# ax-le/nn-fac

Hardware: AMD Instinct MI355X
Metric: HALS NMF outer iterations/s (100000x2000 rank-50 row blocks per second) (higher is better)
Workload: dtype f32; 1 GPU; NMF hals beta=2, 100000x2000 rank 50 per GPU (configs[1] of BASELINE.json), deterministic (alpha=inf, delta=0.01, maxiter=100); rows_total=100000, cols=2000, rank=50, rows_per_rank=100000, parallelism=single GPU, cost_evaluation=streaming kernel (nnf_frob_resid_f32)

## Files before the change

include/nnfac_hip.h:

```cpp
#ifndef NNFAC_HIP_H
#define NNFAC_HIP_H

#include <stddef.h>
#include <stdint.h>

#ifdef __cplusplus
extern "C" {
#endif

#define NNF_OK 0
#define NNF_ERR_ARG (-1)
#define NNF_ERR_LAUNCH (-2)
#define NNF_ERR_UNSUPPORTED (-3)
#define NNF_ERR_WORKSPACE (-4)
#define NNF_ERR_DEVICE (-5)

#define NNF_MAX_RANK 128

#define NNF_HALS_SPARSITY 1u
#define NNF_HALS_NORMALIZE 2u
#define NNF_HALS_NONZERO 4u

typedef struct nnf_ctx nnf_ctx;

// ... 4 lines not shown
#define NNF_HALS_ST_WORDS 8

int nnf_version(void);
size_t nnf_build_flags(char* buf, size_t cap);
const char* nnf_status_string(int status);

int nnf_ctx_create(nnf_ctx** out_ctx, int device, size_t workspace_bytes);
int nnf_ctx_destroy(nnf_ctx* ctx);
size_t nnf_ctx_workspace_bytes(const nnf_ctx* ctx);
int nnf_ctx_set_scratch(nnf_ctx* ctx, void* device_buf, size_t bytes);

int nnf_ctx_set_probe(nnf_ctx* ctx, void* ev_begin, void* ev_end);
#define NNF_PROBE_XTY 0
#define NNF_PROBE_XHT 1
#define NNF_PROBE_COST 2
#define NNF_PROBE_HALS 3
#define NNF_PROBE_MU_LEFT 4
#define NNF_PROBE_MU_RIGHT 5
#define NNF_PROBE_MTTKRP 6
#define NNF_PROBE_COUNT 7
int nnf_ctx_set_probe_kernel(nnf_ctx* ctx, int kernel_id);
int nnf_ctx_set_probe_ring(nnf_ctx* ctx, void* const* events, int npairs);
int nnf_ctx_probe_ring_count(const nnf_ctx* ctx);

typedef struct nnf_comm nnf_comm;
int nnf_comm_unique_id(void* id_out_128_bytes);
int nnf_comm_create(nnf_comm** out_comm, nnf_ctx* ctx, int nranks, int rank, const void* id_128_bytes);
int nnf_comm_destroy(nnf_comm* comm);
int nnf_comm_size(const nnf_comm* comm);
int nnf_comm_rank(const nnf_comm* comm);
int nnf_allreduce_f32(nnf_comm* comm, float* buf, int64_t count, void* stream);
int nnf_allreduce_f64(nnf_comm* comm, double* buf, int64_t count, void* stream);

int nnf_gram_f32(nnf_ctx* ctx, const float* A, int r, int64_t K, int64_t lda, float* G, int64_t ldg, void* stream);
int nnf_gram_f64_f32(nnf_ctx* ctx, const float* A, int r, int64_t K, int64_t lda, float* G, int64_t ldg, double* G64, void* stream);

int nnf_xht_f32(nnf_ctx* ctx, const float* X, int64_t m, int64_t n, int64_t ldx, const float* V, int r, int64_t ldv,
                float* out, int64_t ldo, void* stream);

int nnf_xty_f32(nnf_ctx* ctx, const float* X, int64_t m, int64_t n, int64_t ldx, const float* Ut, int r, int64_t ldu,
                float* out, int64_t ldo, void* stream);

int nnf_frob_resid_f32(nnf_ctx* ctx, const float* X, int64_t m, int64_t n, int64_t ldx, const float* Ut, int64_t ldu,
                       const float* V, int64_t ldv, int r, double* out_f64, void* stream);

int nnf_nmf_gram_cost_f32(nnf_ctx* ctx, const float* V, int64_t ldv, const float* UtM, int64_t ldm, const float* UtU, const float* UtU_b,
                          int64_t ldg, int r, int64_t n, const double* normx2_f64, double* out_f64, void* stream);
int nnf_nmf_gram_cost_cal_f32(nnf_ctx* ctx, const float* V, int64_t ldv, const float* UtM, int64_t ldm, const float* UtU,
                              const float* UtU_b, int64_t ldg, int r, int64_t n, const double* normx2_f64, double sigma_a,
                              double bias_a, double* out_f64, void* stream);
int nnf_nmf_gram_cost_g64_f32(nnf_ctx* ctx, const float* V, int64_t ldv, const float* UtM, int64_t ldm, const float* UtU,
                              const double* UtU64, int64_t ldg, int r, int64_t n, const double* normx2_f64, double sigma_a,
                              double bias_a, double sigma_g, double* out_f64, void* stream);

int nnf_hals_solve_f32(nnf_ctx* ctx, const float* UtM, int64_t ldm, const float* UtU, int64_t ldg, float* V, int64_t ldv,
                       int r, int64_t ncols, int max_sweeps, double delta, float sparsity, unsigned flags,
                       double* status_f64, void* stream);

int nnf_hals_solve_cross_f32(nnf_ctx* ctx, const float* UtM, int64_t ldm, const float* UtU_a, const float* UtU_b, int64_t ldg,
                             const float* V_in, int64_t ldvi, float* V_out, int64_t ldvo, int r, int64_t ncols, int max_sweeps,
                             double delta, float sparsity, unsigned flags, double* status_f64, void* stream);

int nnf_hals_solve_continue_f32(nnf_ctx* ctx, const float* UtM, int64_t ldm, const float* UtU, int64_t ldg, float* V,
                                int64_t ldv, int r, int64_t ncols, int sweeps_done, int max_sweeps, double delta,
                                float sparsity, unsigned flags, double* status_f64, void* stream);

int nnf_hals_sweeps_f32(nnf_ctx* ctx, const float* UtM, int64_t ldm, const float* UtU, int64_t ldg, float* V, int64_t ldv,
                        int r, int64_t ncols, int nsweeps, float sparsity, unsigned flags, double* nodelta_f64,
                        float* snapshots, int64_t snap_stride, void* stream);

int nnf_hals_sweeps_ex_f32(nnf_ctx* ctx, const float* UtM, int64_t ldm, const float* UtU, int64_t ldg, float* V, int64_t ldv,
                           int r, int64_t ncols, int nsweeps, int sweeps_done, float sparsity, unsigned flags,
                           double* nodelta_f64, float* snapshots, int64_t snap_stride, int snap_first, const float* resid_in,
                           float* resid_out, void* stream);
int nnf_hals_resid_floats(nnf_ctx* ctx, int r, int64_t ncols, int64_t* floats_out);

int nnf_hals_row_update_f32(nnf_ctx* ctx, const float* UtM, int64_t ldm, const float* UtU, int64_t ldg, float* V, int64_t ldv, int r,
                            int64_t ncols, int k, float sparsity, unsigned flags, double* out2_f64, void* stream);
int nnf_hals_row_scale_f32(nnf_ctx* ctx, float* V, int64_t ldv, int64_t ncols, int k, const double* normsq_f64, int64_t ncols_total,
                           void* stream);

int nnf_hals_resident_columns(nnf_ctx* ctx, int r, int64_t* columns_out);

int nnf_hals_stop_restore_f32(nnf_ctx* ctx, const double* sums_f64, int nsweeps, int head, int budget, double delta, float* V,
                              int64_t ldv, int r, int64_t ncols, const float* snapshots, int64_t snap_stride,
                              double* status_f64, void* stream);

int nnf_mu_left_f32(nnf_ctx* ctx, const float* X, int64_t m, int64_t n, int64_t ldx, const float* Ut, int64_t ldu,
                    const float* V, int64_t ldv, int r, double beta, float* Ut_out, int64_t lduo, void* stream);

int nnf_mu_left_kl_cost_f32(nnf_ctx* ctx, const float* X, int64_t m, int64_t n, int64_t ldx, const float* Ut, int64_t ldu,
                            const float* V, int64_t ldv, int r, float* Ut_out, int64_t lduo, double* cost_f64, void* stream);

int nnf_mu_right_f32(nnf_ctx* ctx, const float* X, int64_t m, int64_t n, int64_t ldx, const float* Ut, int64_t ldu,
                     const float* V, int64_t ldv, int r, double beta, float* V_out, int64_t ldvo, void* stream);

int nnf_mu_right_accum_f32(nnf_ctx* ctx, const float* X, int64_t m, int64_t n, int64_t ldx, const float* Ut, int64_t ldu,
                           const float* V, int64_t ldv, int r, double beta, float* num, int64_t ldnum, float* den,
                           int64_t ldden, double* den_vec_f64, void* stream);
int nnf_mu_apply_f32(nnf_ctx* ctx, const float* F, int64_t ldf, int r, int64_t cols, const float* num, int64_t ldnum,
                     const float* den, int64_t ldden, const double* den_vec_f64, double beta, float* out, int64_t ldo,
                     void* stream);

int nnf_mu_ratio_f32(nnf_ctx* ctx, const float* X, int64_t m, int64_t n, int64_t ldx, const float* Ut, int64_t ldu,
                     const float* V, int64_t ldv, int r, double beta, float* R1, float* R2, int64_t ldr, void* stream);

// ... 42 lines not shown
```

nn_fac_amd/_lib.py:

```python
import ctypes as C
import os

from .utils.errors import EngineError

_HERE = os.path.dirname(os.path.abspath(__file__))
LIB_PATH = os.environ.get("NNF_LIBRARY") or os.path.join(_HERE, "libnnfac_hip.so")

_i64, _i32, _u32 = C.c_int64, C.c_int, C.c_uint
_p, _f32, _f64 = C.c_void_p, C.c_float, C.c_double

SIGNATURES = {
    "nnf_version": (_i32, []),
    "nnf_build_flags": (C.c_size_t, [C.c_char_p, C.c_size_t]),
    "nnf_status_string": (C.c_char_p, [_i32]),
    "nnf_ctx_create": (_i32, [C.POINTER(_p), _i32, C.c_size_t]),
    "nnf_ctx_destroy": (_i32, [_p]),
    "nnf_ctx_workspace_bytes": (C.c_size_t, [_p]),
    "nnf_comm_unique_id": (_i32, [_p]),
    "nnf_comm_create": (_i32, [C.POINTER(_p), _p, _i32, _i32, _p]),
    "nnf_comm_destroy": (_i32, [_p]),
    "nnf_comm_size": (_i32, [_p]),
    "nnf_comm_rank": (_i32, [_p]),
    "nnf_allreduce_f32": (_i32, [_p, _p, _i64, _p]),
    "nnf_allreduce_f64": (_i32, [_p, _p, _i64, _p]),
    "nnf_gram_f32": (_i32, [_p, _p, _i32, _i64, _i64, _p, _i64, _p]),
    "nnf_xht_f32": (_i32, [_p, _p, _i64, _i64, _i64, _p, _i32, _i64, _p, _i64, _p]),
    "nnf_xty_f32": (_i32, [_p, _p, _i64, _i64, _i64, _p, _i32, _i64, _p, _i64, _p]),
    "nnf_ctx_set_scratch": (_i32, [_p, _p, C.c_size_t]),
    "nnf_frob_resid_f32": (_i32, [_p, _p, _i64, _i64, _i64, _p, _i64, _p, _i64, _i32, _p, _p]),
    "nnf_nmf_gram_cost_f32": (_i32, [_p, _p, _i64, _p, _i64, _p, _p, _i64, _i32, _i64, _p, _p, _p]),
    "nnf_nmf_gram_cost_cal_f32": (_i32, [_p, _p, _i64, _p, _i64, _p, _p, _i64, _i32, _i64, _p, _f64, _f64, _p, _p]),
    "nnf_nmf_gram_cost_g64_f32": (_i32, [_p, _p, _i64, _p, _i64, _p, _p, _i64, _i32, _i64, _p, _f64, _f64, _f64, _p, _p]),
    "nnf_gram_f64_f32": (_i32, [_p, _p, _i32, _i64, _i64, _p, _i64, _p, _p]),
    "nnf_hals_solve_f32": (_i32, [_p, _p, _i64, _p, _i64, _p, _i64, _i32, _i64, _i32, _f64, _f32, _u32, _p, _p]),
    "nnf_hals_solve_cross_f32": (_i32, [_p, _p, _i64, _p, _p, _i64, _p, _i64, _p, _i64, _i32, _i64, _i32, _f64, _f32, _u32, _p,
                                        _p]),
    "nnf_hals_solve_continue_f32": (_i32, [_p, _p, _i64, _p, _i64, _p, _i64, _i32, _i64, _i32, _i32, _f64, _f32, _u32, _p,
                                           _p]),
    "nnf_hals_resident_columns": (_i32, [_p, _i32, C.POINTER(_i64)]),
    "nnf_hals_row_update_f32": (_i32, [_p, _p, _i64, _p, _i64, _p, _i64, _i32, _i64, _i32, _f32, _u32, _p, _p]),
    "nnf_hals_row_scale_f32": (_i32, [_p, _p, _i64, _i64, _i32, _p, _i64, _p]),
    "nnf_hals_stop_restore_f32": (_i32, [_p, _p, _i32, _i32, _i32, _f64, _p, _i64, _i32, _i64, _p, _i64, _p, _p]),
    "nnf_hals_sweeps_f32": (_i32, [_p, _p, _i64, _p, _i64, _p, _i64, _i32, _i64, _i32, _f32, _u32, _p, _p, _i64, _p]),
    "nnf_hals_sweeps_ex_f32": (_i32, [_p, _p, _i64, _p, _i64, _p, _i64, _i32, _i64, _i32, _i32, _f32, _u32, _p, _p, _i64, _i32,
                                      _p, _p, _p]),
    "nnf_hals_resid_floats": (_i32, [_p, _i32, _i64, C.POINTER(_i64)]),
    "nnf_ctx_set_probe": (_i32, [_p, _p, _p]),
    "nnf_ctx_set_probe_kernel": (_i32, [_p, _i32]),
    "nnf_ctx_set_probe_ring": (_i32, [_p, C.POINTER(_p), _i32]),
    "nnf_ctx_probe_ring_count": (_i32, [_p]),
    "nnf_mu_left_f32": (_i32, [_p, _p, _i64, _i64, _i64, _p, _i64, _p, _i64, _i32, _f64, _p, _i64, _p]),
    "nnf_mu_left_kl_cost_f32": (_i32, [_p, _p, _i64, _i64, _i64, _p, _i64, _p, _i64, _i32, _p, _i64, _p, _p]),
    "nnf_mu_right_f32": (_i32, [_p, _p, _i64, _i64, _i64, _p, _i64, _p, _i64, _i32, _f64, _p, _i64, _p]),
    "nnf_mu_right_accum_f32": (_i32, [_p, _p, _i64, _i64, _i64, _p, _i64, _p, _i64, _i32, _f64, _p, _i64, _p, _i64, _p, _p]),
    "nnf_ttm3_f32": (_i32, [_p, _p, _i64, _i64, _i64, _p, _i64, _i32, _i32, _p, _p]),
    "nnf_ntd_core_pg_f32": (_i32, [_p, _p, _p, _p, _p, _p, _i32, _i32, _i32, _f64, _f64, _i32, _f64, _p, _p]),
    "nnf_mu_ratio_f32": (_i32, [_p, _p, _i64, _i64, _i64, _p, _i64, _p, _i64, _i32, _f64, _p, _p, _i64, _p]),
    "nnf_mu_apply_f32": (_i32, [_p, _p, _i64, _i32, _i64, _p, _i64, _p, _i64, _p, _f64, _p, _i64, _p]),
    "nnf_mu_left_num_f32": (_i32, [_p, _p, _i64, _i64, _i64, _p, _i64, _p, _i64, _i32, _p, _i64, _p]),
    "nnf_small_gemm_f32": (_i32, [_p, _p, _i64, _i32, _i32, _p, _i64, _i64, _p, _i64, _p]),
    "nnf_deep_kl_apply_f32": (_i32, [_p, _p, _i64, _i32, _i64, _p, _i64, _p, _p, _i64, _f64, _p, _i64, _p]),
    "nnf_betadiv_f32": (_i32, [_p, _p, _i64, _i64, _i64, _p, _i64, _p, _i64, _i32, _f64, _p, _p]),
    "nnf_mttkrp3_f32": (_i32, [_p, _p, _i64, _i64, _i64, _p, _i64, _p, _i64, _p, _i64, _i32, _i32, _p, _i64, _p]),
    "nnf_mttkrp3_from_partial_f32": (_i32, [_p, _p, _i64, _i64, _p, _i64, _i32, _i32, _p, _i64, _p]),
    "nnf_cp3_partial_cost_f32": (_i32, [_p, _p, _i64, _i64, _i64, _p, _i64, _p, _i64, _p, _i64, _i32, _p, _p, _p]),
    "nnf_cp3_betadiv_f32": (_i32, [_p, _p, _i64, _i64, _i64, _p, _i64, _p, _i64, _p, _i64, _i32, _f64, _p, _p]),
    "nnf_dot_f32": (_i32, [_p, _p, _i64, _p, _i64, _i64, _i64, _p, _p]),
    "nnf_hadamard_f32": (_i32, [_p, _p, _p, _p, _i64, _p]),
}

_lib = None


def load():
    global _lib
    if _lib is not None:
        return _lib
    if not os.path.exists(LIB_PATH):
        raise EngineError(
            f"{LIB_PATH} not found: build it with `python -c 'import __graft_entry__ as g; g.build()'` "
            "or `make -C nn_fac_amd/csrc -j8` (there is no CPU fallback)")
    try:
        lib = C.CDLL(LIB_PATH)
    except OSError as e:
        raise EngineError(f"cannot load {LIB_PATH}: {e}") from e
# ... 12 lines not shown
```

nn_fac_amd/csrc/nnf_api.hip:

```cpp
#include "nnf_internal.h"
#include <new>

#include <map>
#include <string>
#include <string.h>

extern "C" int nnf_version(void) { return 101; }

static std::map<std::string, std::string>& build_flag_registry() {
    static std::map<std::string, std::string> r;
    return r;
}
void nnf_register_build_flags(const char* unit, const char* flags) { build_flag_registry()[unit] = flags; }

extern "C" size_t nnf_build_flags(char* buf, size_t cap) {
    std::string all;
    for (const auto& kv : build_flag_registry()) {
        if (!all.empty()) all += "; ";
        all += kv.first + ": " + kv.second;
    }
    if (buf && cap > 0) {
        const size_t n = all.size() < cap - 1 ? all.size() : cap - 1;
        memcpy(buf, all.data(), n);
        buf[n] = 0;
// ... 114 lines not shown
    for (int64_t e = (int64_t)blockIdx.x * 256 + threadIdx.x; e < total; e += (int64_t)gridDim.x * 256) {
        const int64_t i = e / cols, j = e - i * cols;
        s += (double)A[i * lda + j] * (double)B[i * ldb + j];
    }
    const double t = nnf_block_sum_f64(s, red);
    if (threadIdx.x == 0) partial[blockIdx.x] = t;
}
__global__ __launch_bounds__(256) void nnf_sum_f64_kernel(const double* __restrict__ partial, int64_t count,
                                                          double* __restrict__ out) {
    __shared__ double red[4];
    double s = 0.0;
    for (int64_t e = threadIdx.x; e < count; e += 8 * 256) {
        double v[8];
#pragma unroll
        for (int u = 0; u < 8; ++u) v[u] = partial[e + 256 * u < count ? e + 256 * u : count - 1];
#pragma unroll
        for (int u = 0; u < 8; ++u) s += (e + 256 * u < count) ? v[u] : 0.0;
    }
    const double t = nnf_block_sum_f64(s, red);
    if (threadIdx.x == 0) out[0] = t;
}

extern "C" int nnf_dot_f32(nnf_ctx* ctx, const float* A, int64_t lda, const float* B, int64_t ldb, int64_t rows,
                           int64_t cols, double* out_f64, void* stream) {
    if (!ctx || !A || !B || !out_f64 || rows < 1 || cols < 1 || lda < cols || ldb < cols) return NNF_ERR_ARG;
    hipStream_t st = (hipStream_t)stream;
    int64_t grid = nnf_cdiv(rows * cols, 256 * 8);
    if (grid > 1024) grid = 1024;
    if (grid < 1) grid = 1;
    nnf_ws_cursor cur(ctx);
    double* partial = (double*)cur.take((size_t)grid * 8);
    if (!partial) return NNF_ERR_WORKSPACE;
    hipLaunchKernelGGL(nnf_dot_kernel, dim3((int)grid), dim3(256), 0, st, A, lda, B, ldb, rows, cols, partial);
    NNF_CHECK_LAUNCH();
    hipLaunchKernelGGL(nnf_sum_f64_kernel, dim3(1), dim3(256), 0, st, partial, grid, out_f64);
    NNF_CHECK_LAUNCH();
    return NNF_OK;
}

__global__ void nnf_hadamard_kernel(const float* __restrict__ A, const float* __restrict__ B, float* __restrict__ C,
                                    int64_t count) {
    for (int64_t e = (int64_t)blockIdx.x * blockDim.x + threadIdx.x; e < count; e += (int64_t)gridDim.x * blockDim.x)
        C[e] = A[e] * B[e];
}
extern "C" int nnf_hadamard_f32(nnf_ctx* ctx, const float* A, const float* B, float* C, int64_t count, void* stream) {
    if (!ctx || !A || !B || !C || count < 1) return NNF_ERR_ARG;
    int64_t grid = nnf_cdiv(count, 256);
    if (grid > 1024) grid = 1024;
    hipLaunchKernelGGL(nnf_hadamard_kernel, dim3((int)grid), dim3(256), 0, (hipStream_t)stream, A, B, C, count);
    NNF_CHECK_LAUNCH();
    return NNF_OK;
}

template <typename GT>
__global__ __launch_bounds__(256) void nnf_gram_cost_kernel(const float* __restrict__ V, int64_t ldv, const float* __restrict__ UtM,
                                                            int64_t ldm, const float* __restrict__ G, const float* __restrict__ G2,
                                                            const double* __restrict__ G64, int64_t ldg, int r, int64_t n,
                                                            double* __restrict__ partial, unsigned* __restrict__ ticket,
                                                            const double* __restrict__ normx2, double* __restrict__ out,
                                                            double sigma_a, double bias_a, int g_global, double sigma_g) {
    extern __shared__ __attribute__((aligned(16))) float gc_sh[];
    GT* gsh = reinterpret_cast<GT*>(gc_sh);
    const GT* gsrc = reinterpret_cast<const GT*>(std::is_same<GT, double>::value ? (const void*)G64 : (const void*)G);
    const GT* g = g_global ? gsrc : gsh;
    const int64_t gs = g_global ? (std::is_same<GT, double>::value ? (int64_t)r : ldg) : r;
    float* vc = gc_sh + (g_global ? (size_t)0 : (size_t)r * r * (sizeof(GT) / 4));
    __shared__ double red[4];
    __shared__ unsigned last;
    if (!g_global)
        for (int e = threadIdx.x; e < r * r; e += 256) {
            const int64_t o = (int64_t)(e / r) * ldg + (e % r);
            if constexpr (std::is_same<GT, double>::value) gsh[e] = G64[e];
            else gsh[e] = G2 ? G[o] * G2[o] : G[o];
        }
    const int tc = threadIdx.x >> 4, t = threadIdx.x & 15;
    const int64_t j = (int64_t)blockIdx.x * 16 + tc;
    for (int a = t; a < r; a += 16) vc[tc * r + a] = (j < n) ? V[(int64_t)a * ldv + j] : 0.f;
    __syncthreads();
    double pA = 0.0, pA2 = 0.0, pB = 0.0, pV2 = 0.0;
    if (j < n) {
        const float* vj = vc + tc * r;
        for (int a = t; a < r; a += 16) {
            const GT* ga = g + (size_t)a * gs;
            double ta = 0.0;
            if (g_global && G2 != nullptr) {
                const float* gb = G2 + (size_t)a * ldg;
                for (int b = 0; b < r; ++b) ta = __builtin_fma((double)((float)ga[b] * gb[b]), (double)vj[b], ta);
            } else
            for (int b = 0; b < r; ++b) ta = __builtin_fma((double)ga[b], (double)vj[b], ta);
            const double va = (double)vj[a], p = va * (double)UtM[(int64_t)a * ldm + j];
            pA += p;
            pA2 = __builtin_fma(p, p, pA2);
            pB = __builtin_fma(va, ta, pB);
            pV2 = __builtin_fma(va, va, pV2);
        }
    }
    const double sA = nnf_block_sum_f64(pA, red), sA2 = nnf_block_sum_f64(pA2, red), sB = nnf_block_sum_f64(pB, red),
                 sV2 = nnf_block_sum_f64(pV2, red);
    if (threadIdx.x == 0) {
        unsigned long long* o = reinterpret_cast<unsigned long long*>(partial) + (size_t)blockIdx.x * 4;
        const double vals[4] = {sA, sA2, sB, sV2};
        for (int i = 0; i < 4; ++i)
            __hip_atomic_store(o + i, __builtin_bit_cast(unsigned long long, vals[i]), __ATOMIC_RELAXED, __HIP_MEMORY_SCOPE_AGENT);
        const unsigned tk = __hip_atomic_fetch_add(ticket, 1u, __ATOMIC_ACQ_REL, __HIP_MEMORY_SCOPE_AGENT);
        last = (tk == gridDim.x - 1u) ? 1u : 0u;
    }
    __syncthreads();
    if (last == 0u) return;
    const int nwg = (int)gridDim.x;
    double s[4] = {0.0, 0.0, 0.0, 0.0};
    const unsigned long long* pp = reinterpret_cast<const unsigned long long*>(partial);
    for (int e = threadIdx.x; e < nwg; e += 256)
#pragma unroll
        for (int i = 0; i < 4; ++i)
            s[i] += __builtin_bit_cast(double, __hip_atomic_load(pp + (size_t)e * 4 + i, __ATOMIC_RELAXED, __HIP_MEMORY_SCOPE_AGENT));
    double tot[4];
#pragma unroll
    for (int i = 0; i < 4; ++i) tot[i] = nnf_block_sum_f64(s[i], red);
    float gm = 0.f;
    for (int e = threadIdx.x; e < r * r; e += 256) {
        float ge = (float)g[(size_t)(e / r) * gs + (e % r)];
        if (g_global && G2 != nullptr) ge *= G2[(size_t)(e / r) * ldg + (e % r)];
        gm = fmaxf(gm, fabsf(ge));
    }
    gm = fmaxf(gm, __shfl_xor(gm, 1, 64));
    gm = fmaxf(gm, __shfl_xor(gm, 2, 64));
    gm = fmaxf(gm, __shfl_xor(gm, 4, 64));
    gm = fmaxf(gm, __shfl_xor(gm, 8, 64));
    gm = fmaxf(gm, __shfl_xor(gm, 16, 64));
    gm = fmaxf(gm, __shfl_xor(gm, 32, 64));
    __shared__ float gmax[4];
    if ((threadIdx.x & 63) == 0) gmax[threadIdx.x >> 6] = gm;
    __syncthreads();
    if (threadIdx.x == 0) {
        gm = fmaxf(fmaxf(gmax[0], gmax[1]), fmaxf(gmax[2], gmax[3]));
        const double cost = normx2[0] - 2.0 * tot[0] + tot[2];
        const double sa = 2.0 * sigma_a * sqrt(tot[1]), sb = sigma_g * (double)gm * tot[3];
        const double est = 4.0 * sqrt(sa * sa + sb * sb) + 2.0 * 2.0 * bias_a * fabs(tot[0]);
        out[0] = cost;
        out[1] = (est <= 5e-4 * cost) ? 0.0 : 1.0;
        out[2] = est;
        __hip_atomic_store(ticket, 0u, __ATOMIC_RELAXED, __HIP_MEMORY_SCOPE_AGENT);
    }
}
static int gram_cost_launch(nnf_ctx* ctx, const float* V, int64_t ldv, const float* UtM, int64_t ldm, const float* UtU,
                            const float* UtU_b, const double* UtU64, int64_t ldg, int r, int64_t n, const double* normx2_f64,
                            double sigma_a, double bias_a, double sigma_g, double* out_f64, void* stream) {
    if (!ctx || !V || !UtM || !UtU || !normx2_f64 || !out_f64 || r < 1 || n < 1 || ldv < n || ldm < n || ldg < r) return NNF_ERR_ARG;
    if (!(sigma_a >= 0.0) || !(bias_a >= 0.0) || !(sigma_g >= 0.0)) return NNF_ERR_ARG;
    if (UtU64 != nullptr && UtU_b != nullptr) return NNF_ERR_ARG;
    const int g_global = r > NNF_MAX_RANK ? 1 : 0;
    hipStream_t st = (hipStream_t)stream;
    const int64_t nwg = nnf_cdiv(n, 16);
    if (nwg > (int64_t)1 << 24) return NNF_ERR_UNSUPPORTED;
    nnf_ws_cursor cur(ctx);
    double* partial = (double*)cur.take((size_t)nwg * 4 * 8);
    if (!partial) return NNF_ERR_WORKSPACE;
    unsigned* ticket = ctx->gc_ticket;
    if (!ticket) return NNF_ERR_WORKSPACE;
    const size_t shm = ((g_global ? (size_t)0 : (size_t)r * r * (UtU64 ? 2 : 1)) + (size_t)16 * r) * 4;
    if (shm > 150 * 1024) return NNF_ERR_UNSUPPORTED;
    if (UtU64) {
        static bool attr = false;
        if (!attr) {
            (void)hipFuncSetAttribute(reinterpret_cast<const void*>(&nnf_gram_cost_kernel<double>), hipFuncAttributeMaxDynamicSharedMemorySize,
                                      150 * 1024);
            attr = true;
        }
        hipLaunchKernelGGL(nnf_gram_cost_kernel<double>, dim3((int)nwg), dim3(256), shm, st, V, ldv, UtM, ldm, UtU, UtU_b, UtU64, ldg, r, n,
                           partial, ticket, normx2_f64, out_f64, sigma_a, bias_a, g_global, sigma_g);
    } else {
        static bool attr = false;
        if (!attr) {
            (void)hipFuncSetAttribute(reinterpret_cast<const void*>(&nnf_gram_cost_kernel<float>), hipFuncAttributeMaxDynamicSharedMemorySize,
                                      96 * 1024);
            attr = true;
        }
        hipLaunchKernelGGL(nnf_gram_cost_kernel<float>, dim3((int)nwg), dim3(256), shm, st, V, ldv, UtM, ldm, UtU, UtU_b, UtU64, ldg, r, n,
                           partial, ticket, normx2_f64, out_f64, sigma_a, bias_a, g_global, sigma_g);
    }
    NNF_CHECK_LAUNCH();
    return NNF_OK;
}
extern "C" int nnf_nmf_gram_cost_f32(nnf_ctx* ctx, const float* V, int64_t ldv, const float* UtM, int64_t ldm, const float* UtU,
                                     const float* UtU_b, int64_t ldg, int r, int64_t n, const double* normx2_f64, double* out_f64,
                                     void* stream) {
    return gram_cost_launch(ctx, V, ldv, UtM, ldm, UtU, UtU_b, nullptr, ldg, r, n, normx2_f64, 6e-8, 0.0, 4e-8, out_f64, stream);
}
extern "C" int nnf_nmf_gram_cost_cal_f32(nnf_ctx* ctx, const float* V, int64_t ldv, const float* UtM, int64_t ldm, const float* UtU,
                                         const float* UtU_b, int64_t ldg, int r, int64_t n, const double* normx2_f64, double sigma_a,
                                         double bias_a, double* out_f64, void* stream) {
    return gram_cost_launch(ctx, V, ldv, UtM, ldm, UtU, UtU_b, nullptr, ldg, r, n, normx2_f64, sigma_a, bias_a, 4e-8, out_f64, stream);
}
extern "C" int nnf_nmf_gram_cost_g64_f32(nnf_ctx* ctx, const float* V, int64_t ldv, const float* UtM, int64_t ldm, const float* UtU,
                                         const double* UtU64, int64_t ldg, int r, int64_t n, const double* normx2_f64, double sigma_a,
                                         double bias_a, double sigma_g, double* out_f64, void* stream) {
    if (!UtU64) return NNF_ERR_ARG;
    return gram_cost_launch(ctx, V, ldv, UtM, ldm, UtU, nullptr, UtU64, ldg, r, n, normx2_f64, sigma_a, bias_a, sigma_g, out_f64, stream);
}
```

nn_fac_amd/engine.py:

```python
import ctypes as C
import os
import threading

import torch

from . import _lib
from .utils import errors as err
from .utils.errors import EngineError

HALS_SPARSITY, HALS_NORMALIZE, HALS_NONZERO = 1, 2, 4
ST_EPS, ST_CNT, ST_EPS0, ST_ERR, ST_WORDS = 0, 1, 2, 3, 8

_engines = {}
_lock = threading.Lock()

MAX_RANK = 128


def check_rank(r, where):
    r = int(r)
    if r > MAX_RANK:
        raise EngineError(f"{where}: rank {r} is above the {MAX_RANK} the Tucker kernels (core contractions, core update) of "
                          f"nn_fac_amd are built for; nmf, ntf, hals_nnls_acc and mu_betadivmin take any rank")

# ... 56 lines not shown
            if out64.dtype != torch.float64 or not out64.is_contiguous() or out64.numel() < r * r or out64.device != A.device:
                raise EngineError("gram: out64 must be a contiguous float64 device tensor of r*r elements")
            _lib.check(self.lib.nnf_gram_f64_f32(self.ctx, _ptr(A), r, K, _ld(A), _ptr(G), _ld(G), _ptr(out64), self._stream()),
                       "nnf_gram_f64_f32")
            return G
        _lib.check(self.lib.nnf_gram_f32(self.ctx, _ptr(A), r, K, _ld(A), _ptr(G), _ld(G), self._stream()),
                   "nnf_gram_f32")
        return G

    def xht(self, X, V, out=None):
        _chk2d(X, "xht X"), _chk2d(V, "xht V")
        m, n = X.shape
        r = V.shape[0]
        if V.shape[1] != n:
            raise EngineError("xht: shape mismatch")
        O = out if out is not None else torch.empty((r, m), dtype=torch.float32, device=X.device)
        _lib.check(self.lib.nnf_xht_f32(self.ctx, _ptr(X), m, n, _ld(X), _ptr(V), r, _ld(V), _ptr(O),
                                        _ld(O), self._stream()), "nnf_xht_f32")
        return O

    def xty(self, X, Ut, out=None):
        _chk2d(X, "xty X"), _chk2d(Ut, "xty Ut")
        m, n = X.shape
        r = Ut.shape[0]
        if Ut.shape[1] != m:
            raise EngineError("xty: shape mismatch")
        O = out if out is not None else torch.empty((r, n), dtype=torch.float32, device=X.device)
        _lib.check(self.lib.nnf_xty_f32(self.ctx, _ptr(X), m, n, _ld(X), _ptr(Ut), r, _ld(Ut), _ptr(O),
                                        _ld(O), self._stream()), "nnf_xty_f32")
        return O

    def frob_resid(self, X, Ut, V, out=None):
        _chk2d(X, "frob X"), _chk2d(Ut, "frob Ut"), _chk2d(V, "frob V")
        m, n = X.shape
        r = Ut.shape[0]
        if Ut.shape[1] != m or V.shape != (r, n):
            raise EngineError("frob_resid: shape mismatch")
        o = out if out is not None else torch.empty(1, dtype=torch.float64, device=X.device)
        self._model_scratch(m, n, r)
        _lib.check(self.lib.nnf_frob_resid_f32(self.ctx, _ptr(X), m, n, _ld(X), _ptr(Ut), _ld(Ut), _ptr(V),
                                               _ld(V), r, _ptr(o), self._stream()), "nnf_frob_resid_f32")
        return o

    def _model_scratch(self, m, n, r):
        if r <= MAX_RANK:
            return
        need = int(m) * ((int(n) + 3) // 4 * 4) * 4
        cur = getattr(self, "_scratch", None)
        if cur is None or cur.numel() < need:
            torch.cuda.current_stream(self.device).synchronize()
            self._scratch = torch.empty(need, dtype=torch.uint8, device=self.device)
            _lib.check(self.lib.nnf_ctx_set_scratch(self.ctx, _ptr(self._scratch), need), "nnf_ctx_set_scratch")

    def gram_cost(self, V, UtM, UtU, normx2, out, UtU_b=None, rounding=None, UtU64=None):
        _chk2d(V, "gram_cost V"), _chk2d(UtM, "gram_cost UtM"), _chk2d(UtU, "gram_cost UtU")
        r, n = V.shape
        if UtM.shape != (r, n) or UtU.shape[0] < r or UtU.shape[1] < r or normx2.dtype != torch.float64 or out.dtype != torch.float64 \
                or out.numel() < 3:
            raise EngineError("gram_cost: shape / dtype mismatch")
        if UtU_b is not None and (UtU_b.shape != UtU.shape or _ld(UtU_b) != _ld(UtU)):
            raise EngineError("gram_cost: the two Grams of a Hadamard pair must share shape and leading dimension")
        sa, ba = (6e-8, 0.0) if rounding is None else (float(rounding[0]), float(rounding[1]))
        if UtU64 is not None and UtU_b is None:
            sg = float(rounding[2]) if rounding is not None and len(rounding) > 2 else 1e-8
            _lib.check(self.lib.nnf_nmf_gram_cost_g64_f32(self.ctx, _ptr(V), _ld(V), _ptr(UtM), _ld(UtM), _ptr(UtU), _ptr(UtU64),
                                                          _ld(UtU), r, n, _ptr(normx2), sa, ba, sg, _ptr(out), self._stream()),
                       "nnf_nmf_gram_cost_g64_f32")
            return out
        _lib.check(self.lib.nnf_nmf_gram_cost_cal_f32(self.ctx, _ptr(V), _ld(V), _ptr(UtM), _ld(UtM), _ptr(UtU),
                                                      _ptr(UtU_b) if UtU_b is not None else None, _ld(UtU), r, n,
                                                      _ptr(normx2), sa, ba, _ptr(out), self._stream()), "nnf_nmf_gram_cost_cal_f32")
        return out

    def cross_rounding(self, X, Ut, blocks=16):
        m = int(X.shape[0])
        full = self.xty(X, Ut).double()
        acc = torch.zeros_like(full)
        step = -(-m // int(blocks))
        step = -(-step // 256) * 256
        for lo in range(0, m, step):
            hi = min(m, lo + step)
            acc += self.xty(X[lo:hi], Ut[:, lo:hi]).double()
        rel = (full - acc) / acc.clamp_min(1e-300)
        rel = torch.where(acc > 0, rel, torch.zeros_like(rel))
        return float(rel.pow(2).mean().sqrt()), abs(float(rel.mean()))

    def gram_rounding(self, Ut, blocks=16):
        r, m = Ut.shape
        full = torch.empty((r, r), dtype=torch.float64, device=Ut.device)
        self.gram(Ut, out64=full)
        acc, part = torch.zeros_like(full), torch.empty_like(full)
        step = -(-m // int(blocks))
        step = -(-step // 256) * 256
        for lo in range(0, m, step):
            self.gram(Ut[:, lo:min(m, lo + step)], out64=part)
            acc += part
        rel = (full - acc) / acc.abs().clamp_min(1e-300)
        rel = torch.where(acc != 0, rel, torch.zeros_like(rel))
        return float(rel.pow(2).mean().sqrt())

    def dot(self, A, B):
        _chk2d(A, "dot A"), _chk2d(B, "dot B")
        o = torch.empty(1, dtype=torch.float64, device=A.device)
        _lib.check(self.lib.nnf_dot_f32(self.ctx, _ptr(A), _ld(A), _ptr(B), _ld(B), A.shape[0], A.shape[1],
                                        _ptr(o), self._stream()), "nnf_dot_f32")
        return o

    def hadamard(self, A, B, out=None):
        A, B = A.contiguous(), B.contiguous()
        Cc = out if out is not None else torch.empty_like(A)
        _lib.check(self.lib.nnf_hadamard_f32(self.ctx, _ptr(A), _ptr(B), _ptr(Cc), A.numel(), self._stream()),
                   "nnf_hadamard_f32")
        return Cc

    @staticmethod
# ... 459 lines not shown
```

nn_fac_amd/nmf.py:

```python
import math
import os
import time
import warnings

import numpy as np
import torch

from .utils import errors as err
from .utils import initialize_factors as init_factors
from . import engine as _engine
from ._convert import device_of, to_dev, to_dev_t, like_input
from . import dist as _dist


def nmf(data, rank, init="random", U_0=None, V_0=None, n_iter_max=100, tol=1e-8,
        update_rule="hals", beta=2,
        sparsity_coefficients=[None, None], fixed_modes=[], normalize=[False, False],
        verbose=False, return_costs=False, deterministic=False, seed=0):
    if min(data.shape) < rank:
        min_data = min(data.shape)
        rank = min_data
        warnings.warn(f"The rank is too high for the input matrix. It was set to {min_data} instead.")

    if deterministic:
# ... 233 lines not shown
                         nranks=_dist.world(group) if _dist.is_sharded(group) else 0)
        if step.get("ident"):
            if float(host[20]) != 0.0:
                raise _IdentityUnreliable()
            c, e = float(host[19]), float(host[21])
            if tol is not None and tol > 0 and last is not None and abs(last[0] - c) < tol + e + last[1]:
                raise _IdentityNearStop()
            last = (c, e)
        pending.pop(0)
        result = (step["Ut"], step["V"])
        if group is not None and update_rule == "hals" and step["nstat"] >= 1 and 0 not in fixed_modes:
            cnt_u = int(host[_engine.ST_CNT]) - 1
            ws.async_ready = ws.last_u_count is not None and abs(cnt_u - ws.last_u_count) <= 4
            ws.last_u_count = cnt_u
        if step.get("async_u"):
            ws.async_hits += 1
            ws.guess_u.value = max(8, min(int(host[_engine.ST_CNT]) - 1 + 4, ws.guess_u.max_chunk))
        stop = bool(retired(step["it"], float(host[19 if step.get("ident") else 16]),
                            [int(host[8 * i + _engine.ST_CNT]) - 1 for i in range(step["nstat"])]))

    def drain():
        if cuda:
            main.synchronize()
            if ws.cost_stream is not None:
                ws.cost_stream.synchronize()

    def fall_back():
        nonlocal overlap, depth, owed, costed, stop
        drain()
        pending.clear()
        ws.safe_solve = True
        overlap, depth, owed, costed = False, PIPELINE_DEPTH, None, None
        warnings.warn("nn_fac_amd: a persistent HALS solve timed out waiting for its workgroups (GPU shared with another "
                      "process?); falling back to chunked launches for the rest of this run")

    owed = None
    costed = None
    iteration = 0
    while iteration < n_iter:
        ws.select(iteration % ws.blocks.shape[0])
        hooks = {}
        if fused_mu and owed is not None:
            hooks["mu_cost_out"] = ws.blocks[owed["slot"]][16:17]
        if overlap and owed is not None:
            hooks["before_v_solve"] = lambda prev=owed: cost_of(prev, ws.cost_stream)
        if overlap and costed is not None:
            hooks["before_u_solve"] = lambda ev=costed["ev"]: main.wait_event(ev)
        Ut, V, nstat = _one_nmf_step_dev(eng, ws, X, rank, Ut, V, update_rule, beta, sparsity_coefficients,
                                         fixed_modes, normalize, deterministic, group=group,
                                         skip_cost=overlap or fused_mu or ident, **hooks)
        step = dict(it=iteration, slot=ws.slot, Ut=Ut, V=V, nstat=nstat, ev=None, async_u=ws.last_step_async, ident=ident)
        ws.sync_next = False
        if ident:
            eng.gram_cost(V, ws.UtM, ws.G2, ws.normx2, ws.block[19:22], rounding=ws.cross_rounding,
                          UtU64=ws.G64 if ws.g64_ok else None)
            _add_sparsity_terms(Ut, V, sparsity_coefficients, ws.block[19:20], group)
            _dist.allreduce_errs_(ws.block, group)
            ws.host[ws.slot].copy_(ws.block, non_blocking=True)
            step["ev"] = main.record_event()
        elif fused_mu:
            if owed is not None:
                _dist.allreduce_cost_(ws.blocks[owed["slot"]], group)
                ws.host[owed["slot"]].copy_(ws.blocks[owed["slot"]], non_blocking=True)
                owed["ev"] = main.record_event()
            owed = step
        elif overlap:
            costed = owed
            owed = step
        elif cuda:
            ws.host[ws.slot].copy_(ws.block, non_blocking=True)
            step["ev"] = main.record_event()
        else:
            ws.host[ws.slot].copy_(ws.block)
        pending.append(step)
        iteration += 1
        try:
            if len(pending) > depth:
                retire()
                if stop:
                    break
            if iteration == n_iter:
                if (overlap or fused_mu) and not stop and owed is not None and owed["ev"] is None:
                    cost_of(owed, main)
                while pending and not stop:
                    retire()
        except _SolveTimedOut:
            failed = pending[0]["it"]
            fall_back()
            Ut, V = result
            iteration = failed
        except _IdentityUnreliable:
            failed = pending[0]["it"]
            drain()
            pending.clear()
            if last is not None and hasattr(retired, "revise_last"):
                scratch = torch.zeros_like(ws.block)
                _step_cost(eng, X, result[0], result[1], update_rule, beta, sparsity_coefficients, scratch, group)
                retired.revise_last(float(scratch[16]))
            last = None
            ws.direct_cost = True
            ident = False
            overlap = (ws.cost_stream is not None
                       and (not _dist.is_sharded(group) or _dist.opt_in("NNF_SHARDED_OVERLAP", group)))
            depth = PIPELINE_DEPTH + (1 if overlap else 0)
            owed = costed = None
            Ut, V = result
            iteration = failed
        except _GuessMissed:
            failed = pending[0]["it"]
            drain()
            pending.clear()
# ... 189 lines not shown
```

Before: 1274 iterations/s.

## Add wide gram-cost kernel and fuse status-block mirror to pinned host

Adds a 1024-thread gram-cost kernel that stages V, UtM and a transposed Gram in shared memory and computes per-column V^T G products in double before reducing. The kernel is enabled by default through an environment switch. The last workgroup now also writes the whole status block straight into pinned host memory with system-scope stores, which removes the separate device-to-host copy and the sparsity/allreduce launches in the non-sparse, single-GPU path. In exchange it uses more shared memory per block, relies on the ordering of system-scope stores for the host to see the data, and in the mirror path substitutes a hard-coded Gram rounding sigma when no 64-bit Gram is supplied.

```diff
diff --git a/include/nnfac_hip.h b/include/nnfac_hip.h
--- a/include/nnfac_hip.h
+++ b/include/nnfac_hip.h
@@ -80,6 +80,10 @@
 int nnf_nmf_gram_cost_g64_f32(nnf_ctx* ctx, const float* V, int64_t ldv, const float* UtM, int64_t ldm, const float* UtU,
                               const double* UtU64, int64_t ldg, int r, int64_t n, const double* normx2_f64, double sigma_a,
                               double bias_a, double sigma_g, double* out_f64, void* stream);
+int nnf_nmf_gram_cost_mirror_f32(nnf_ctx* ctx, const float* V, int64_t ldv, const float* UtM, int64_t ldm, const float* UtU,
+                                 const double* UtU64, int64_t ldg, int r, int64_t n, const double* normx2_f64, double sigma_a,
+                                 double bias_a, double sigma_g, double* out_f64, const double* block_f64, double* host_f64,
+                                 int words, void* stream);
 
 int nnf_hals_solve_f32(nnf_ctx* ctx, const float* UtM, int64_t ldm, const float* UtU, int64_t ldg, float* V, int64_t ldv,
                        int r, int64_t ncols, int max_sweeps, double delta, float sparsity, unsigned flags,
diff --git a/nn_fac_amd/_lib.py b/nn_fac_amd/_lib.py
--- a/nn_fac_amd/_lib.py
+++ b/nn_fac_amd/_lib.py
@@ -31,6 +31,8 @@
     "nnf_nmf_gram_cost_f32": (_i32, [_p, _p, _i64, _p, _i64, _p, _p, _i64, _i32, _i64, _p, _p, _p]),
     "nnf_nmf_gram_cost_cal_f32": (_i32, [_p, _p, _i64, _p, _i64, _p, _p, _i64, _i32, _i64, _p, _f64, _f64, _p, _p]),
     "nnf_nmf_gram_cost_g64_f32": (_i32, [_p, _p, _i64, _p, _i64, _p, _p, _i64, _i32, _i64, _p, _f64, _f64, _f64, _p, _p]),
+    "nnf_nmf_gram_cost_mirror_f32": (_i32, [_p, _p, _i64, _p, _i64, _p, _p, _i64, _i32, _i64, _p, _f64, _f64, _f64, _p, _p, _p, _i32,
+                                            _p]),
     "nnf_gram_f64_f32": (_i32, [_p, _p, _i32, _i64, _i64, _p, _i64, _p, _p]),
     "nnf_hals_solve_f32": (_i32, [_p, _p, _i64, _p, _i64, _p, _i64, _i32, _i64, _i32, _f64, _f32, _u32, _p, _p]),
     "nnf_hals_solve_cross_f32": (_i32, [_p, _p, _i64, _p, _p, _i64, _p, _i64, _p, _i64, _i32, _i64, _i32, _f64, _f32, _u32, _p,
diff --git a/nn_fac_amd/csrc/nnf_api.hip b/nn_fac_amd/csrc/nnf_api.hip
--- a/nn_fac_amd/csrc/nnf_api.hip
+++ b/nn_fac_amd/csrc/nnf_api.hip
@@ -190,13 +190,66 @@
     return NNF_OK;
 }
 
+struct nnf_gc_mirror {
+    const double* src;
+    double* dst;
+    int words;
+};
+
+__device__ __forceinline__ void nnf_gram_cost_finish(const double* __restrict__ partial, unsigned* __restrict__ ticket,
+                                                     const double* __restrict__ normx2, double* out, double sigma_a, double bias_a,
+                                                     double sigma_g, float gm, double* red, nnf_gc_mirror mirror) {
+    __shared__ float gmax[16];
+    __shared__ double fin[3];
+    const int nwg = (int)gridDim.x, nw = (int)((blockDim.x + 63) >> 6);
+    double s[4] = {0.0, 0.0, 0.0, 0.0};
+    const unsigned long long* pp = reinterpret_cast<const unsigned long long*>(partial);
+    if (threadIdx.x < 256)
+        for (int e = threadIdx.x; e < nwg; e += 256)
+#pragma unroll
+            for (int i = 0; i < 4; ++i)
+                s[i] += __builtin_bit_cast(double, __hip_atomic_load(pp + (size_t)e * 4 + i, __ATOMIC_RELAXED, __HIP_MEMORY_SCOPE_AGENT));
+    double tot[4];
+#pragma unroll
+    for (int i = 0; i < 4; ++i) tot[i] = nnf_block_sum_f64(s[i], red);
+    gm = fmaxf(gm, __shfl_xor(gm, 1, 64));
+    gm = fmaxf(gm, __shfl_xor(gm, 2, 64));
+    gm = fmaxf(gm, __shfl_xor(gm, 4, 64));
+    gm = fmaxf(gm, __shfl_xor(gm, 8, 64));
+    gm = fmaxf(gm, __shfl_xor(gm, 16, 64));
+    gm = fmaxf(gm, __shfl_xor(gm, 32, 64));
+    if ((threadIdx.x & 63) == 0) gmax[threadIdx.x >> 6] = gm;
+    __syncthreads();
+    if (threadIdx.x == 0) {
+        for (int i = 1; i < nw; ++i) gm = fmaxf(gm, gmax[i]);
+        const double cost = normx2[0] - 2.0 * tot[0] + tot[2];
+        const double sa = 2.0 * sigma_a * sqrt(tot[1]), sb = sigma_g * (double)gm * tot[3];
+        const double est = 4.0 * sqrt(sa * sa + sb * sb) + 2.0 * 2.0 * bias_a * fabs(tot[0]);
+        const double flag = (est <= 5e-4 * cost) ? 0.0 : 1.0;
+        out[0] = fin[0] = cost;
+        out[1] = fin[1] = flag;
+        out[2] = fin[2] = est;
+        __hip_atomic_store(ticket, 0u, __ATOMIC_RELAXED, __HIP_MEMORY_SCOPE_AGENT);
+    }
+    if (mirror.dst != nullptr) {
+        __syncthreads();
+        if ((int)threadIdx.x < mirror.words) {
+            const double* sp = mirror.src + threadIdx.x;
+            const long long k = sp - out;
+            const double v = (k >= 0 && k < 3) ? fin[k] : *sp;
+            __hip_atomic_store(reinterpret_cast<unsigned long long*>(mirror.dst) + threadIdx.x, __builtin_bit_cast(unsigned long long, v),
+                               __ATOMIC_RELAXED, __HIP_MEMORY_SCOPE_SYSTEM);
+        }
+    }
+}
+
 template <typename GT>
 __global__ __launch_bounds__(256) void nnf_gram_cost_kernel(const float* __restrict__ V, int64_t ldv, const float* __restrict__ UtM,
                                                             int64_t ldm, const float* __restrict__ G, const float* __restrict__ G2,
                                                             const double* __restrict__ G64, int64_t ldg, int r, int64_t n,
                                                             double* __restrict__ partial, unsigned* __restrict__ ticket,
                                                             const double* __restrict__ normx2, double* __restrict__ out,
-                                                            double sigma_a, double bias_a, int g_global, double sigma_g) {
+                                                            double sigma_a, double bias_a, int g_global, double sigma_g, nnf_gc_mirror mirror) {
     extern __shared__ __attribute__((aligned(16))) float gc_sh[];
     GT* gsh = reinterpret_cast<GT*>(gc_sh);
     const GT* gsrc = reinterpret_cast<const GT*>(std::is_same<GT, double>::value ? (const void*)G64 : (const void*)G);
@@ -245,48 +298,95 @@
     }
     __syncthreads();
     if (last == 0u) return;
-    const int nwg = (int)gridDim.x;
-    double s[4] = {0.0, 0.0, 0.0, 0.0};
-    const unsigned long long* pp = reinterpret_cast<const unsigned long long*>(partial);
-    for (int e = threadIdx.x; e < nwg; e += 256)
-#pragma unroll
-        for (int i = 0; i < 4; ++i)
-            s[i] += __builtin_bit_cast(double, __hip_atomic_load(pp + (size_t)e * 4 + i, __ATOMIC_RELAXED, __HIP_MEMORY_SCOPE_AGENT));
-    double tot[4];
-#pragma unroll
-    for (int i = 0; i < 4; ++i) tot[i] = nnf_block_sum_f64(s[i], red);
     float gm = 0.f;
     for (int e = threadIdx.x; e < r * r; e += 256) {
         float ge = (float)g[(size_t)(e / r) * gs + (e % r)];
         if (g_global && G2 != nullptr) ge *= G2[(size_t)(e / r) * ldg + (e % r)];
         gm = fmaxf(gm, fabsf(ge));
     }
-    gm = fmaxf(gm, __shfl_xor(gm, 1, 64));
-    gm = fmaxf(gm, __shfl_xor(gm, 2, 64));
-    gm = fmaxf(gm, __shfl_xor(gm, 4, 64));
-    gm = fmaxf(gm, __shfl_xor(gm, 8, 64));
-    gm = fmaxf(gm, __shfl_xor(gm, 16, 64));
-    gm = fmaxf(gm, __shfl_xor(gm, 32, 64));
-    __shared__ float gmax[4];
-    if ((threadIdx.x & 63) == 0) gmax[threadIdx.x >> 6] = gm;
-    __syncthreads();
+    nnf_gram_cost_finish(partial, ticket, normx2, out, sigma_a, bias_a, sigma_g, gm, red, mirror);
+}
+
+template <typename GT>
+__global__ __launch_bounds__(1024) void nnf_gram_cost_wide_kernel(const float* __restrict__ V, int64_t ldv, const float* __restrict__ UtM,
+                                                                  int64_t ldm, const float* __restrict__ G, const float* __restrict__ G2,
+                                                                  const double* __restrict__ G64, int64_t ldg, int r, int64_t n,
+                                                                  double* __restrict__ partial, unsigned* __restrict__ ticket,
+                                                                  const double* __restrict__ normx2, double* __restrict__ out,
+                                                                  double sigma_a, double bias_a, double sigma_g, nnf_gc_mirror mirror) {
+    extern __shared__ __attribute__((aligned(16))) float gc_sh[];
+    double* ta_s = reinterpret_cast<double*>(gc_sh);
+    GT* gT = reinterpret_cast<GT*>(ta_s + (size_t)16 * r);
+    float* vc = reinterpret_cast<float*>(gT + (size_t)r * r);
+    float* um = vc + (size_t)16 * r;
+    __shared__ double red[16];
+    __shared__ unsigned last;
+    for (int e = threadIdx.x; e < r * r; e += 1024) {
+        const int a = e / r, b = e - a * r;
+        const int64_t o = (int64_t)a * ldg + b;
+        if constexpr (std::is_same<GT, double>::value) gT[b * r + a] = G64[e];
+        else gT[b * r + a] = G2 ? G[o] * G2[o] : G[o];
+    }
+    const int tc = threadIdx.x & 15, aq = threadIdx.x >> 4;
+    const int64_t j = (int64_t)blockIdx.x * 16 + tc;
+    for (int a = aq; a < r; a += 64) {
+        vc[a * 16 + tc] = (j < n) ? V[(int64_t)a * ldv + j] : 0.f;
+        um[a * 16 + tc] = (j < n) ? UtM[(int64_t)a * ldm + j] : 0.f;
+    }
+    __syncthreads();
+    if (j < n) {
+        for (int a = aq; a < r; a += 64) {
+            double ta = 0.0;
+            int b = 0;
+            for (; b + 8 <= r; b += 8) {
+                GT gv[8];
+                float vv[8];
+#pragma unroll
+                for (int u = 0; u < 8; ++u) { gv[u] = gT[(b + u) * r + a]; vv[u] = vc[(b + u) * 16 + tc]; }
+#pragma unroll
+                for (int u = 0; u < 8; ++u) ta = __builtin_fma((double)gv[u], (double)vv[u], ta);
+            }
+            for (; b < r; ++b) ta = __builtin_fma((double)gT[b * r + a], (double)vc[b * 16 + tc], ta);
+            ta_s[a * 16 + tc] = ta;
+        }
+    }
+    __syncthreads();
+    double pA = 0.0, pA2 = 0.0, pB = 0.0, pV2 = 0.0;
+    if (threadIdx.x < 256) {
+        const int c2 = threadIdx.x >> 4, t = threadIdx.x & 15;
+        if ((int64_t)blockIdx.x * 16 + c2 < n)
+            for (int a = t; a < r; a += 16) {
+                const double va = (double)vc[a * 16 + c2], u = (double)um[a * 16 + c2], p = va * u;
+                pA = __builtin_fma(va, u, pA);
+                pA2 = __builtin_fma(p, p, pA2);
+                pB = __builtin_fma(va, ta_s[a * 16 + c2], pB);
+                pV2 = __builtin_fma(va, va, pV2);
+            }
+    }
+    const double sA = nnf_block_sum_f64(pA, red), sA2 = nnf_block_sum_f64(pA2, red), sB = nnf_block_sum_f64(pB, red),
+                 sV2 = nnf_block_sum_f64(pV2, red);
     if (threadIdx.x == 0) {
-        gm = fmaxf(fmaxf(gmax[0], gmax[1]), fmaxf(gmax[2], gmax[3]));
-        const double cost = normx2[0] - 2.0 * tot[0] + tot[2];
-        const double sa = 2.0 * sigma_a * sqrt(tot[1]), sb = sigma_g * (double)gm * tot[3];
-        const double est = 4.0 * sqrt(sa * sa + sb * sb) + 2.0 * 2.0 * bias_a * fabs(tot[0]);
-        out[0] = cost;
-        out[1] = (est <= 5e-4 * cost) ? 0.0 : 1.0;
-        out[2] = est;
-        __hip_atomic_store(ticket, 0u, __ATOMIC_RELAXED, __HIP_MEMORY_SCOPE_AGENT);
-    }
+        unsigned long long* o = reinterpret_cast<unsigned long long*>(partial) + (size_t)blockIdx.x * 4;
+        const double vals[4] = {sA, sA2, sB, sV2};
+        for (int i = 0; i < 4; ++i)
+            __hip_atomic_store(o + i, __builtin_bit_cast(unsigned long long, vals[i]), __ATOMIC_RELAXED, __HIP_MEMORY_SCOPE_AGENT);
+        const unsigned tk = __hip_atomic_fetch_add(ticket, 1u, __ATOMIC_ACQ_REL, __HIP_MEMORY_SCOPE_AGENT);
+        last = (tk == gridDim.x - 1u) ? 1u : 0u;
+    }
+    __syncthreads();
+    if (last == 0u) return;
+    float gm = 0.f;
+    for (int e = threadIdx.x; e < r * r; e += 1024) gm = fmaxf(gm, fabsf((float)gT[e]));
+    nnf_gram_cost_finish(partial, ticket, normx2, out, sigma_a, bias_a, sigma_g, gm, red, mirror);
 }
 static int gram_cost_launch(nnf_ctx* ctx, const float* V, int64_t ldv, const float* UtM, int64_t ldm, const float* UtU,
                             const float* UtU_b, const double* UtU64, int64_t ldg, int r, int64_t n, const double* normx2_f64,
-                            double sigma_a, double bias_a, double sigma_g, double* out_f64, void* stream) {
+                            double sigma_a, double bias_a, double sigma_g, double* out_f64, void* stream,
+                            nnf_gc_mirror mirror = {nullptr, nullptr, 0}) {
     if (!ctx || !V || !UtM || !UtU || !normx2_f64 || !out_f64 || r < 1 || n < 1 || ldv < n || ldm < n || ldg < r) return NNF_ERR_ARG;
     if (!(sigma_a >= 0.0) || !(bias_a >= 0.0) || !(sigma_g >= 0.0)) return NNF_ERR_ARG;
     if (UtU64 != nullptr && UtU_b != nullptr) return NNF_ERR_ARG;
+    if (mirror.dst != nullptr && (!mirror.src || mirror.words < 1 || mirror.words > 256)) return NNF_ERR_ARG;
     const int g_global = r > NNF_MAX_RANK ? 1 : 0;
     hipStream_t st = (hipStream_t)stream;
     const int64_t nwg = nnf_cdiv(n, 16);
@@ -296,27 +396,28 @@
     if (!partial) return NNF_ERR_WORKSPACE;
     unsigned* ticket = ctx->gc_ticket;
     if (!ticket) return NNF_ERR_WORKSPACE;
-    const size_t shm = ((g_global ? (size_t)0 : (size_t)r * r * (UtU64 ? 2 : 1)) + (size_t)16 * r) * 4;
+    const size_t gbytes = (size_t)r * r * (UtU64 ? 8 : 4);
+    const size_t shm_wide = gbytes + (size_t)16 * r * (8 + 4 + 4);
+    const char* wide_env = getenv("NNF_GRAM_COST_WIDE");
+    const int wide_on = wide_env ? atoi(wide_env) : 1;
+    const bool wide = !g_global && wide_on && shm_wide <= 150 * 1024;
+    const size_t shm = wide ? shm_wide : (g_global ? (size_t)0 : gbytes) + (size_t)16 * r * 4;
     if (shm > 150 * 1024) return NNF_ERR_UNSUPPORTED;
-    if (UtU64) {
-        static bool attr = false;
-        if (!attr) {
-            (void)hipFuncSetAttribute(reinterpret_cast<const void*>(&nnf_gram_cost_kernel<double>), hipFuncAttributeMaxDynamicSharedMemorySize,
-                                      150 * 1024);
-            attr = true;
-        }
-        hipLaunchKernelGGL(nnf_gram_cost_kernel<double>, dim3((int)nwg), dim3(256), shm, st, V, ldv, UtM, ldm, UtU, UtU_b, UtU64, ldg, r, n,
-                           partial, ticket, normx2_f64, out_f64, sigma_a, bias_a, g_global, sigma_g);
-    } else {
-        static bool attr = false;
-        if (!attr) {
-            (void)hipFuncSetAttribute(reinterpret_cast<const void*>(&nnf_gram_cost_kernel<float>), hipFuncAttributeMaxDynamicSharedMemorySize,
-                                      96 * 1024);
-            attr = true;
-        }
-        hipLaunchKernelGGL(nnf_gram_cost_kernel<float>, dim3((int)nwg), dim3(256), shm, st, V, ldv, UtM, ldm, UtU, UtU_b, UtU64, ldg, r, n,
-                           partial, ticket, normx2_f64, out_f64, sigma_a, bias_a, g_global, sigma_g);
-    }
+#define NNF_GC_LAUNCH(KERNEL, THREADS, ...)                                                                                       \
+    do {                                                                                                                        \
+        static bool attr = false;                                                                                               \
+        if (!attr) {                                                                                                            \
+            (void)hipFuncSetAttribute(reinterpret_cast<const void*>(&KERNEL), hipFuncAttributeMaxDynamicSharedMemorySize, 150 * 1024); \
+            attr = true;                                                                                                        \
+        }                                                                                                                       \
+        hipLaunchKernelGGL(KERNEL, dim3((int)nwg), dim3(THREADS), shm, st, V, ldv, UtM, ldm, UtU, UtU_b, UtU64, ldg, r, n, partial, \
+                           ticket, normx2_f64, out_f64, sigma_a, bias_a, __VA_ARGS__);                                          \
+    } while (0)
+    if (wide && UtU64) NNF_GC_LAUNCH(nnf_gram_cost_wide_kernel<double>, 1024, sigma_g, mirror);
+    else if (wide) NNF_GC_LAUNCH(nnf_gram_cost_wide_kernel<float>, 1024, sigma_g, mirror);
+    else if (UtU64) NNF_GC_LAUNCH(nnf_gram_cost_kernel<double>, 256, g_global, sigma_g, mirror);
+    else NNF_GC_LAUNCH(nnf_gram_cost_kernel<float>, 256, g_global, sigma_g, mirror);
+#undef NNF_GC_LAUNCH
     NNF_CHECK_LAUNCH();
     return NNF_OK;
 }
@@ -336,3 +437,12 @@
     if (!UtU64) return NNF_ERR_ARG;
     return gram_cost_launch(ctx, V, ldv, UtM, ldm, UtU, nullptr, UtU64, ldg, r, n, normx2_f64, sigma_a, bias_a, sigma_g, out_f64, stream);
 }
+
+extern "C" int nnf_nmf_gram_cost_mirror_f32(nnf_ctx* ctx, const float* V, int64_t ldv, const float* UtM, int64_t ldm, const float* UtU,
+                                            const double* UtU64, int64_t ldg, int r, int64_t n, const double* normx2_f64,
+                                            double sigma_a, double bias_a, double sigma_g, double* out_f64, const double* block_f64,
+                                            double* host_f64, int words, void* stream) {
+    if (!block_f64 || !host_f64 || words < 1 || words > 256) return NNF_ERR_ARG;
+    return gram_cost_launch(ctx, V, ldv, UtM, ldm, UtU, nullptr, UtU64, ldg, r, n, normx2_f64, sigma_a, bias_a, UtU64 ? sigma_g : 4e-8,
+                            out_f64, stream, {block_f64, host_f64, words});
+}
diff --git a/nn_fac_amd/engine.py b/nn_fac_amd/engine.py
--- a/nn_fac_amd/engine.py
+++ b/nn_fac_amd/engine.py
@@ -132,7 +132,7 @@
             self._scratch = torch.empty(need, dtype=torch.uint8, device=self.device)
             _lib.check(self.lib.nnf_ctx_set_scratch(self.ctx, _ptr(self._scratch), need), "nnf_ctx_set_scratch")
 
-    def gram_cost(self, V, UtM, UtU, normx2, out, UtU_b=None, rounding=None, UtU64=None):
+    def gram_cost(self, V, UtM, UtU, normx2, out, UtU_b=None, rounding=None, UtU64=None, mirror=None):
         _chk2d(V, "gram_cost V"), _chk2d(UtM, "gram_cost UtM"), _chk2d(UtU, "gram_cost UtU")
         r, n = V.shape
         if UtM.shape != (r, n) or UtU.shape[0] < r or UtU.shape[1] < r or normx2.dtype != torch.float64 or out.dtype != torch.float64 \
@@ -141,6 +141,19 @@
         if UtU_b is not None and (UtU_b.shape != UtU.shape or _ld(UtU_b) != _ld(UtU)):
             raise EngineError("gram_cost: the two Grams of a Hadamard pair must share shape and leading dimension")
         sa, ba = (6e-8, 0.0) if rounding is None else (float(rounding[0]), float(rounding[1]))
+        if mirror is not None:
+            block, host = mirror
+            if UtU_b is not None or block.dtype != torch.float64 or host.dtype != torch.float64 or not block.is_contiguous() \
+                    or not host.is_contiguous() or not host.is_pinned() or host.numel() != block.numel() or block.numel() > 256 \
+                    or block.device != V.device:
+                raise EngineError("gram_cost: the mirror is a contiguous float64 block of <= 256 words and a pinned host tensor of its size")
+            sg = float(rounding[2]) if rounding is not None and len(rounding) > 2 else 1e-8
+            _lib.check(self.lib.nnf_nmf_gram_cost_mirror_f32(self.ctx, _ptr(V), _ld(V), _ptr(UtM), _ld(UtM), _ptr(UtU),
+                                                             _ptr(UtU64) if UtU64 is not None else None, _ld(UtU), r, n,
+                                                             _ptr(normx2), sa, ba, sg, _ptr(out), _ptr(block),
+                                                             C.c_void_p(host.data_ptr()), block.numel(), self._stream()),
+                       "nnf_nmf_gram_cost_mirror_f32")
+            return out
         if UtU64 is not None and UtU_b is None:
             sg = float(rounding[2]) if rounding is not None and len(rounding) > 2 else 1e-8
             _lib.check(self.lib.nnf_nmf_gram_cost_g64_f32(self.ctx, _ptr(V), _ld(V), _ptr(UtM), _ld(UtM), _ptr(UtU), _ptr(UtU64),
diff --git a/nn_fac_amd/nmf.py b/nn_fac_amd/nmf.py
--- a/nn_fac_amd/nmf.py
+++ b/nn_fac_amd/nmf.py
@@ -309,11 +309,13 @@
         step = dict(it=iteration, slot=ws.slot, Ut=Ut, V=V, nstat=nstat, ev=None, async_u=ws.last_step_async, ident=ident)
         ws.sync_next = False
         if ident:
+            mirrored = not (sparsity_coefficients[0] or sparsity_coefficients[1]) and not _dist.is_sharded(group)
             eng.gram_cost(V, ws.UtM, ws.G2, ws.normx2, ws.block[19:22], rounding=ws.cross_rounding,
-                          UtU64=ws.G64 if ws.g64_ok else None)
-            _add_sparsity_terms(Ut, V, sparsity_coefficients, ws.block[19:20], group)
-            _dist.allreduce_errs_(ws.block, group)
-            ws.host[ws.slot].copy_(ws.block, non_blocking=True)
+                          UtU64=ws.G64 if ws.g64_ok else None, mirror=(ws.block, ws.host[ws.slot]) if mirrored else None)
+            if not mirrored:
+                _add_sparsity_terms(Ut, V, sparsity_coefficients, ws.block[19:20], group)
+                _dist.allreduce_errs_(ws.block, group)
+                ws.host[ws.slot].copy_(ws.block, non_blocking=True)
             step["ev"] = main.record_event()
         elif fused_mu:
             if owed is not None:
```

Result: no change. 1276 iterations/s, median of 6 (+0.2%).
